# IvanPopov/video-flow-ml

Measured on AMD Instinct MI355X. Metric: flow-fields/sec @1080p seq5 MOF_sintel, higher is better.
Workload: dtype mixed (per-layer MFMA count, f32 accumulate): {"corr": 1, "update_block.encoder.convf1": 1, "update_block.encoder.convf2": 1, "update_block.gru.convq1.iter": "2a", "update_block.gru.convzr1.iter": 1, "update_block.gru.convzr2.iter": 1, "update_block.mask.0": 1, "update_block.mask.2": 1, "update_bloc

## Files before the change

include/vfml.h:

```cpp
#ifndef VFML_H
#define VFML_H
#include <stddef.h>
#include <stdint.h>

#ifdef __cplusplus
extern "C" {
#endif

#define VFML_ABI_VERSION 27

enum {
  VFML_EPI_NONE = 0,
  VFML_EPI_RELU = 1,
  VFML_EPI_TANH = 2,
  VFML_EPI_SIGMOID = 3,
  VFML_EPI_TANH_RELU = 4,
  VFML_EPI_GRU_ZR = 5,
  VFML_EPI_GRU_Q = 6,
  VFML_EPI_ADD_AUX = 7,
};

enum { VFML_FMT_F32 = 0, VFML_FMT_S16 = 1,
       VFML_FMT_F16 = 2 };

// ... 91 lines not shown
int vfml_avgpool2x2(const float* x, int n, int h, int w, int c, float* out, void* stream);

int vfml_corr_lookup(const float* const* pyr, const int32_t* hl, const int32_t* wl,
                     const int32_t* ld, int levels, int radius, int nmaps, int q_per_map,
                     const float* coords, int ld_coords, float* out, int ld_out, int out_fmt, int vol_fmt, int vol_tile,
                     void* stream);
#define VFML_VOL_F16_LEVELS(m) (0x100 | (m))

int vfml_corr_lookup_indirect(const float* const* table, const int32_t* hl, const int32_t* wl, const int32_t* ld,
                              int levels, int radius, int nmaps, int q_per_map, const float* coords, int ld_coords,
                              float* out, int ld_out, int out_fmt, int vol_fmt, int vol_tile, void* stream);
int vfml_corr_lookup_indirect_bidir(const float* const* table, const int32_t* hl, const int32_t* wl, const int32_t* ld,
                                    int levels, int radius, int nmaps, int q_per_map, const float* coords, int ld_coords,
                                    int dir_coords, float* out, int ld_out, int dir_out, int dir_tab, int out_fmt, int vol_fmt,
                                    int vol_tile, void* stream);
int vfml_ptr_table_set(void* table, const void* const* ptrs, int n, void* stream);

int vfml_corr_level0_ensure(const vfml_conv_desc* d, const void* w_hi, const void* w_lo, int kp, float w_scale, int in_fmt,
                            int out_fmt, int k_order, const void* const* cells, int centres, int dirs, int dir_cells,
                            const float* coords, int ld_coords, int dir_coords, int h, int w, int radius, int vol_tile,
                            uint32_t* counter, void* stream);

typedef struct vfml_corr_level_desc {
  const vfml_conv_desc* d;
  const void* w_hi;
  const void* w_lo;
  int32_t kp;
  float w_scale;
  int32_t out_fmt, level, h, w;
} vfml_corr_level_desc;
// ... 155 lines not shown
```

video-flow-ml_amd/vfml/csrc/flow_ops.hip:

```cpp
#include <stdlib.h>
#include "vfml_common.h"
#include "corr_window.h"

namespace {

constexpr int MAX_LEVELS = 6;
constexpr int MAX_MAPS = 8;
constexpr int MAX_RADIUS = 4;
constexpr int PATCH = 2 * MAX_RADIUS + 2;
#ifndef VFML_LOOKUP_WAVES
#define VFML_LOOKUP_WAVES 4
#endif
constexpr int LOOKUP_WAVES = VFML_LOOKUP_WAVES;
constexpr int FIXED_LEVELS = 4;
static_assert(FIXED_LEVELS == 4, "corr_lookup_fixed_kernel selects among four levels");

struct LookupArgs {
  const float* pyr[MAX_MAPS][MAX_LEVELS];
  const float* const* table;
  int hl[MAX_LEVELS], wl[MAX_LEVELS], ld[MAX_LEVELS];
  int levels, radius, nq, q_per_map;
  const float* coords; int ld_coords;
  float* out; int ld_out;
  int out16;
// ... 212 lines not shown
      for (int h = 0; h < 2; ++h) {
        const int c = lane * 8 + 4 * h;
        const f32x4 w = h ? v1 : v0;
        if (c + 3 < nout && (((uintptr_t)(o + 4 * h)) & 15u) == 0) {
          *reinterpret_cast<f32x4*>(o + 4 * h) = w;
        } else {
#pragma unroll
          for (int k = 0; k < 4; ++k)
            if (c + k < nout) o[4 * h + k] = w[k];
        }
      }
    }
  }
}

__global__ void coords_init_kernel(f32x4* __restrict__ coords, int h, int w, int64_t total) {
  for (int64_t p = (int64_t)blockIdx.x * blockDim.x + threadIdx.x; p < total; p += (int64_t)gridDim.x * blockDim.x) {
    const int x = (int)(p % w);
    const int y = (int)((p / w) % h);
    f32x4 v = {(float)x, (float)y, (float)x, (float)y};
    coords[p] = v;
  }
}

__global__ void flow_rows7_kernel(const f32x4* __restrict__ flow, int w, int64_t total, char* __restrict__ rows) {
  for (int64_t i = (int64_t)blockIdx.x * blockDim.x + threadIdx.x; i < total * 4; i += (int64_t)gridDim.x * blockDim.x) {
    const int64_t p = i >> 2;
    const int u = (int)(i & 3);
    const int x = (int)(p % w);
    f32x4 t0 = {0.f, 0.f, 0.f, 0.f}, t1 = {0.f, 0.f, 0.f, 0.f};
// ... 188 lines not shown
               "vfml_window_seed: rows >= 1, cols a multiple of 4, rows * cols / 4 <= 2^30");
  VFML_REQUIRE(ld_state % 4 == 0 && h_off >= 0 && mf_off >= 0 && h_off % 4 == 0 && mf_off % 4 == 0 && h_off + cols <= ld_state &&
               mf_off + cols <= ld_state && (h_off + cols <= mf_off || mf_off + cols <= h_off),
               "vfml_window_seed: the two column blocks lie apart inside a state row, at multiples of 4 floats");
  VFML_REQUIRE(ld_ctx >= cols && ld_ctx % 4 == 0, "vfml_window_seed: ld_ctx=%d (>= cols, a multiple of 4)", ld_ctx);
  const int quads = cols / 4;
  hipLaunchKernelGGL(window_seed_kernel, dim3(grid_for((int64_t)rows * quads, 256), ncentres), dim3(256), 0,
                     reinterpret_cast<hipStream_t>(stream), reinterpret_cast<const int64_t*>(cells), rows, quads, state,
                     ld_state, h_off, mf_off, ld_ctx);
  return vfml_check_launch("vfml_window_seed");
}

static int corr_lookup_impl(const float* const* pyr, const float* const* table, const int32_t* hl, const int32_t* wl,
                            const int32_t* ld, int levels, int radius, int nmaps, int q_per_map, const float* coords,
                            int ld_coords, float* out, int ld_out, int out_fmt, int vol_fmt, int vol_tile, void* stream,
                            int dir_maps = 0, int dir_coords = 0, int dir_out = 0, int dir_tab = 0);

extern "C" int vfml_corr_lookup(const float* const* pyr, const int32_t* hl, const int32_t* wl, const int32_t* ld,
                                int levels, int radius, int nmaps, int q_per_map, const float* coords, int ld_coords,
                                float* out, int ld_out, int out_fmt, int vol_fmt, int vol_tile, void* stream) {
  VFML_REQUIRE(pyr, "vfml_corr_lookup: null pointer");
  return corr_lookup_impl(pyr, nullptr, hl, wl, ld, levels, radius, nmaps, q_per_map, coords, ld_coords, out, ld_out, out_fmt,
                          vol_fmt, vol_tile, stream);
}

extern "C" int vfml_corr_lookup_indirect(const float* const* table, const int32_t* hl, const int32_t* wl, const int32_t* ld,
                                         int levels, int radius, int nmaps, int q_per_map, const float* coords,
                                         int ld_coords, float* out, int ld_out, int out_fmt, int vol_fmt, int vol_tile, void* stream) {
  VFML_REQUIRE(table && (reinterpret_cast<uintptr_t>(table) & 7u) == 0, "vfml_corr_lookup_indirect: null / misaligned table");
  return corr_lookup_impl(nullptr, table, hl, wl, ld, levels, radius, nmaps, q_per_map, coords, ld_coords, out, ld_out,
                          out_fmt, vol_fmt, vol_tile, stream);
// ... 1 lines not shown

extern "C" int vfml_corr_lookup_indirect_bidir(const float* const* table, const int32_t* hl, const int32_t* wl, const int32_t* ld,
                                               int levels, int radius, int nmaps, int q_per_map, const float* coords,
                                               int ld_coords, int dir_coords, float* out, int ld_out, int dir_out, int dir_tab,
                                               int out_fmt, int vol_fmt, int vol_tile, void* stream) {
  VFML_REQUIRE(table && (reinterpret_cast<uintptr_t>(table) & 7u) == 0, "vfml_corr_lookup_indirect_bidir: null / misaligned table");
  VFML_REQUIRE(nmaps >= 1 && 2 * nmaps <= MAX_MAPS, "vfml_corr_lookup_indirect_bidir: nmaps=%d out of [1,%d]", nmaps, MAX_MAPS / 2);
  VFML_REQUIRE(dir_coords >= 0 && dir_coords + 2 <= ld_coords && dir_out >= 0 && (out_fmt != VFML_FMT_S16 || dir_out % 8 == 0),
               "vfml_corr_lookup_indirect_bidir: dir_coords within a coords row, dir_out >= 0 (a multiple of 8 floats for split rows)");
  VFML_REQUIRE(dir_tab >= nmaps && (dir_tab + nmaps) * levels <= MAX_TABLE,
               "vfml_corr_lookup_indirect_bidir: dir_tab=%d (the second direction's first map in the table) out of range", dir_tab);
  return corr_lookup_impl(nullptr, table, hl, wl, ld, levels, radius, 2 * nmaps, q_per_map, coords, ld_coords, out, ld_out,
                          out_fmt, vol_fmt, vol_tile, stream, nmaps, dir_coords, dir_out, dir_tab);
}

static int corr_lookup_impl(const float* const* pyr, const float* const* table, const int32_t* hl, const int32_t* wl,
                            const int32_t* ld, int levels, int radius, int nmaps, int q_per_map, const float* coords,
                            int ld_coords, float* out, int ld_out, int out_fmt, int vol_fmt, int vol_tile, void* stream,
                            int dir_maps, int dir_coords, int dir_out, int dir_tab) {
  VFML_REQUIRE(nmaps >= 1 && nmaps <= MAX_MAPS && q_per_map > 0, "vfml_corr_lookup: nmaps=%d out of [1,%d] or empty maps", nmaps, MAX_MAPS);
  const int nq = nmaps * q_per_map;
  VFML_REQUIRE(out_fmt == VFML_FMT_F32 || out_fmt == VFML_FMT_S16, "vfml_corr_lookup: bad out_fmt");
  int v16mask = vol_fmt == VFML_FMT_F16 ? 15 : ((vol_fmt & ~15) == VFML_VOL_F16_LEVELS(0) ? (vol_fmt & 15) : (vol_fmt == VFML_FMT_F32 ? 0 : -1));
  if (v16mask > 0 && levels >= 1 && levels <= FIXED_LEVELS) {
    v16mask &= (1 << levels) - 1;
    if (v16mask) v16mask |= 15 & ~((1 << levels) - 1);
  }
  VFML_REQUIRE(v16mask == 0 || ((radius == 3 || radius == 4) && levels <= FIXED_LEVELS &&
                                (v16mask == 15 || v16mask == 14 || v16mask == 12 || v16mask == 8)),
               "vfml_corr_lookup: vol_fmt is VFML_FMT_F32, or (radius 3 / 4, at most %d levels) VFML_FMT_F16 or "
               "VFML_VOL_F16_LEVELS(m) with m = levels 1-3, 2-3 or 3", FIXED_LEVELS);
  VFML_REQUIRE(hl && wl && ld && coords && out, "vfml_corr_lookup: null pointer");
  VFML_REQUIRE(levels >= 1 && levels <= MAX_LEVELS, "vfml_corr_lookup: levels=%d out of [1,%d]", levels, MAX_LEVELS);
  VFML_REQUIRE(radius >= 1 && radius <= MAX_RADIUS, "vfml_corr_lookup: radius=%d out of [1,%d]", radius, MAX_RADIUS);
// ... 19 lines not shown
  }
  for (int l = levels; l < MAX_LEVELS; ++l) a.hl[l] = a.wl[l] = a.ld[l] = 0;
  a.tws = vol_tile & 15; a.ths = (vol_tile >> 4) & 15; a.qw = wl[0];
  VFML_REQUIRE(vol_tile >= 0 && vol_tile < 256 && a.tws <= 6 && a.ths <= 6, "vfml_corr_lookup: vol_tile = tws + 16 * ths with tws, ths <= 6");
  if (vol_tile) {
    VFML_REQUIRE(q_per_map == hl[0] * wl[0], "vfml_corr_lookup: a tiled volume orders its rows by the level-0 grid (q_per_map == hl[0] * wl[0])");
    for (int l = 0; l < levels; ++l)
      VFML_REQUIRE((int64_t)ld[l] >= (int64_t)(((hl[l] - 1) >> a.ths) + 1) * (((wl[l] - 1) >> a.tws) + 1) << (a.tws + a.ths),
                   "vfml_corr_lookup: ld[%d]=%d is less than the whole tiles of a %d x %d level", l, ld[l], wl[l], hl[l]);
  }
  a.levels = levels; a.radius = radius; a.nq = nq; a.q_per_map = q_per_map;
  a.coords = coords; a.ld_coords = ld_coords; a.out = out; a.ld_out = ld_out;
  a.dir_maps = dir_maps; a.dir_coords = dir_coords; a.dir_out = dir_out; a.dir_tab = dir_tab;
  const dim3 grid((nq + LOOKUP_WAVES - 1) / LOOKUP_WAVES), block(64 * LOOKUP_WAVES);
  hipStream_t st = reinterpret_cast<hipStream_t>(stream);
  if (a.vol16) {
    const int m = a.vol16;
#define VFML_LOOKUP16(RR, OO)                                                                                  \
  do {                                                                                                          \
    if (m == 15) hipLaunchKernelGGL((corr_lookup_fixed_kernel<RR, OO, 15>), grid, block, 0, st, a);             \
    else if (m == 14) hipLaunchKernelGGL((corr_lookup_fixed_kernel<RR, OO, 14>), grid, block, 0, st, a);        \
    else if (m == 12) hipLaunchKernelGGL((corr_lookup_fixed_kernel<RR, OO, 12>), grid, block, 0, st, a);        \
    else hipLaunchKernelGGL((corr_lookup_fixed_kernel<RR, OO, 8>), grid, block, 0, st, a);                      \
  } while (0)
    if (radius == 4) {
      if (a.out16) VFML_LOOKUP16(4, true);
      else VFML_LOOKUP16(4, false);
    } else {
      if (a.out16) VFML_LOOKUP16(3, true);
      else VFML_LOOKUP16(3, false);
// ... 169 lines not shown
```

video-flow-ml_amd/vfml/hip.py:

```python
import ctypes
import os
import subprocess
from ctypes import POINTER, c_char_p, c_double, c_float, c_int, c_int32, c_int64, c_void_p

import torch

_HERE = os.path.dirname(os.path.abspath(__file__))
LIB_PATH = os.environ.get("VFML_LIB") or os.path.join(_HERE, "libvfml_hip.so")
CSRC = os.path.join(_HERE, "csrc")
SOURCES = ["api.hip", "conv_gemm.hip", "conv_gemm_split.hip", "corr_ensure.hip", "conv_gemm_tapx.hip", "conv_split_plan.hip", "stem.hip", "flow_half.hip", "enc_conv.hip", "norm_pool.hip", "flow_ops.hip", "effects.hip", "correct.hip", "render.hip", "text.hip", "turbulence.hip", "resize.hip", "jpeg.hip", "jpeg_decode.hip", "jpeg_decode_sync.hip", "deflate.hip", "attention.hip", "dwconv.hip", "twins.hip", "warm_start.hip"]

STATS_ROWS_F32, STATS_ROWS_S16 = 128, 32
EPI_NONE, EPI_RELU, EPI_TANH, EPI_SIGMOID, EPI_TANH_RELU, EPI_GRU_ZR, EPI_GRU_Q, EPI_ADD_AUX = range(8)
FMT_F32, FMT_S16, FMT_F16 = 0, 1, 2


def vol_f16_levels(mask):
    return 0x100 | mask


def _vol_mask(vol_fmt, levels):
    return (15 if vol_fmt == FMT_F16 else (vol_fmt & 15 if vol_fmt & 0x100 else 0)) & ((1 << levels) - 1)

KORDER_TAP, KORDER_CBLOCK, KORDER_CBLOCK64 = 0, 1, 2
# ... 115 lines not shown
    L.vfml_instnorm_finalize.argtypes = [c_void_p, c_int, c_int, c_int, c_int, c_float, c_void_p, c_void_p, c_int64, c_void_p]
    L.vfml_instnorm_finalize_workspace_bytes.restype = c_int64
    L.vfml_instnorm_finalize_workspace_bytes.argtypes = [c_int, c_int]
    L.vfml_stem7x7s2_chunks.argtypes = [c_int, c_int]
    L.vfml_stem7x7s2.argtypes = [c_void_p, c_int, c_int, c_int, c_void_p, c_void_p, c_float, c_void_p, c_void_p, c_void_p, c_void_p]
    L.vfml_instnorm_apply.argtypes = [c_void_p, c_void_p, c_void_p, c_void_p, c_int, c_int, c_int, c_void_p, c_int, c_void_p]
    L.vfml_avgpool2x2.argtypes = [c_void_p, c_int, c_int, c_int, c_int, c_void_p, c_void_p]
    L.vfml_corr_lookup.argtypes = [POINTER(c_void_p), POINTER(c_int32), POINTER(c_int32), POINTER(c_int32),
                                   c_int, c_int, c_int, c_int, c_void_p, c_int, c_void_p, c_int, c_int, c_int, c_int, c_void_p]
    L.vfml_corr_lookup_indirect.argtypes = [c_void_p, POINTER(c_int32), POINTER(c_int32), POINTER(c_int32),
                                            c_int, c_int, c_int, c_int, c_void_p, c_int, c_void_p, c_int, c_int, c_int, c_int,
                                            c_void_p]
    L.vfml_corr_lookup_indirect_bidir.argtypes = [c_void_p, POINTER(c_int32), POINTER(c_int32), POINTER(c_int32),
                                                  c_int, c_int, c_int, c_int, c_void_p, c_int, c_int, c_void_p, c_int, c_int,
                                                  c_int, c_int, c_int, c_int, c_void_p]
    L.vfml_ptr_table_set.argtypes = [c_void_p, POINTER(c_void_p), c_int, c_void_p]
    L.vfml_corr_level0_ensure.argtypes = L.vfml_conv2d_split.argtypes[:5] + [c_int, c_int, c_int] + [
        c_void_p, c_int, c_int, c_int, c_void_p, c_int, c_int, c_int, c_int, c_int, c_int, c_void_p, c_void_p]
    L.vfml_corr_levels_ensure.argtypes = [POINTER(CorrLevelDesc), c_int, c_int, c_int, c_void_p, c_int, c_int, c_int, c_void_p,
                                          c_int, c_int, c_int, c_int, c_int, c_int, c_void_p, c_void_p]
    L.vfml_window_seed.argtypes = [c_void_p, c_int, c_int, c_int, c_void_p, c_int, c_int, c_int, c_int, c_void_p]
    L.vfml_tapsum3x3_update.argtypes = [c_void_p, c_int, c_void_p, c_int, c_int, c_int, c_int, ctypes.c_int64, c_void_p, c_void_p,
                                        c_int, c_void_p, c_int, c_int, c_void_p]
    L.vfml_conv3x3_c64.argtypes = [c_void_p, c_int, c_int, c_int, c_int, c_void_p, c_void_p, c_int, c_float, c_void_p, c_void_p,
                                   c_int, c_void_p, c_void_p]
    L.vfml_flow_half.argtypes = [c_void_p, c_int, c_int, c_int, c_void_p, c_int, c_float, c_void_p, c_void_p, c_int, c_float,
                                 c_void_p, c_void_p, c_int, c_void_p]
    L.vfml_coords_init.argtypes = [c_void_p, c_int, c_int, c_int, c_void_p]
    L.vfml_flow_rows7.argtypes = [c_void_p, c_int, c_int, c_int, c_void_p, c_void_p]
    L.vfml_tapsum3x3.argtypes = [c_void_p, c_int, c_void_p, c_int, c_int, c_int, c_void_p, c_int, ctypes.c_int64, c_void_p]
# ... 62 lines not shown
    L.vfml_inflate_chunks.argtypes = [c_void_p, c_int64, c_void_p, c_int, c_int, c_int64, ctypes.c_uint32, c_void_p, c_void_p,
                                      c_void_p, c_void_p, c_void_p]
    L.vfml_convex_upsample.argtypes = [c_void_p, c_int, c_void_p, c_int, c_int, c_int, c_void_p, c_void_p]
    for name in EXPORTS:
        getattr(L, name)
    if L.vfml_abi_version() != 27:
        raise RuntimeError("libvfml_hip.so ABI version mismatch")
    _lib = L
    return L


EXPORTS = [
    "vfml_conv2d", "vfml_conv2d_split", "vfml_conv2d_variant", "vfml_conv2d_split_variant", "vfml_conv2d_split_variant_at", "vfml_split_f16", "vfml_to_s16", "vfml_softmax_rows_s16", "vfml_softmax_rows_f16", "vfml_attention_plane_workspace_bytes", "vfml_attention_plane_f16", "vfml_attention_bank_planes_f16", "vfml_axpy_f32", "vfml_dwconv2d", "vfml_gelu_rows", "vfml_layernorm_rows", "vfml_window_attention", "vfml_attention_shared_keys", "vfml_transpose_to_s16", "vfml_add_to_s16",
    "vfml_transpose_split_f16", "vfml_frames_to_nhwc4", "vfml_instnorm_workspace_bytes", "vfml_instnorm_stats",
    "vfml_instnorm_apply", "vfml_instnorm_finalize", "vfml_instnorm_finalize_workspace_bytes", "vfml_avgpool2x2", "vfml_corr_lookup", "vfml_corr_lookup_indirect", "vfml_corr_lookup_indirect_bidir",
    "vfml_ptr_table_set", "vfml_corr_level0_ensure", "vfml_corr_levels_ensure", "vfml_window_seed", "vfml_coords_update", "vfml_coords_init", "vfml_tapsum3x3", "vfml_tapsum3x3_update", "vfml_flow_rows7", "vfml_flow_half", "vfml_conv3x3_c64",
    "vfml_flow_forward_interpolate_workspace_bytes", "vfml_flow_forward_interpolate",
    "vfml_convex_upsample", "vfml_stem7x7s2", "vfml_stem7x7s2_chunks", "vfml_flow_lod", "vfml_flow_encode", "vfml_taa_blend", "vfml_flow_quality_map", "vfml_flow_correct_workspace_bytes", "vfml_flow_correct",
    "vfml_flow_colorize", "vfml_compose_frame", "vfml_flow_decode", "vfml_flow_diff_overlay", "vfml_text_draw",
    "vfml_flow_turbulence_workspace_bytes", "vfml_flow_turbulence_map", "vfml_resize_u8",
    "vfml_jpeg_workspace_bytes", "vfml_jpeg_scan_capacity", "vfml_jpeg_encode_rgb",
    "vfml_jpeg_sampled_workspace_bytes", "vfml_jpeg_sampled_scan_capacity", "vfml_jpeg_encode_rgb_sampled",
    "vfml_jpeg_decode_workspace_bytes", "vfml_jpeg_decode_rgb",
    "vfml_jpeg_decode_sync_workspace_bytes", "vfml_jpeg_decode_rgb_sync",
    "vfml_jpeg_decode_sampled_workspace_bytes", "vfml_jpeg_decode_rgb_sampled",
    "vfml_jpeg_decode_sync_sampled_workspace_bytes", "vfml_jpeg_decode_rgb_sync_sampled",
    "vfml_deflate_capacity", "vfml_deflate_workspace_bytes", "vfml_deflate_huffman",
    "vfml_inflate_workspace_bytes", "vfml_inflate_chunks",
    "vfml_last_error", "vfml_abi_version",
]
# ... 415 lines not shown
        d.out, d.ldo = _ptr(_dev(volume)), ldo
        d.epilogue, d.split, d.out_scale = EPI_NONE, 0, out_scale
        d.flags = {3: 0, 2: CONV_MFMA2, 1: CONV_MFMA1}[mfma]
        lv = lvs[i]
        lv.d = ctypes.pointer(d)
        lv.w_hi, lv.w_lo, lv.kp, lv.w_scale = weight.hi.data_ptr(), weight.lo.data_ptr(), weight.kp, weight.scale
        lv.out_fmt, lv.level, lv.h, lv.w = FMT_F32, level, hl, wl
    order = levels[0][1].order
    _check(lib().vfml_corr_levels_ensure(lvs, len(levels), in_fmt, order, c_void_p(cells.data_ptr()), centres, ndirs, dir_cells,
                                         _ptr(_dev(coords), coords_off), ld_coords, dir_coords, h, w, radius, vol_tile,
                                         c_void_p(counters.data_ptr()) if counters is not None else None, _stream()),
           "vfml_corr_levels_ensure")


SEED_NONE, SEED_LOAD, SEED_STORE = 0, 1, 2


def window_seed(cells, ncentres, rows, cols, state, ld_state, h_off, mf_off, ld_ctx):
    if not (cells.is_cuda and cells.dtype == torch.int64 and cells.numel() >= 3 * ncentres):
        raise ValueError("window_seed: cells must be an int64 device tensor, three per centre frame")
    _check(lib().vfml_window_seed(c_void_p(cells.data_ptr()), ncentres, rows, cols, _ptr(_dev(state)), ld_state, h_off, mf_off,
                                  ld_ctx, _stream()), "vfml_window_seed")


def corr_lookup(pyrs, hl, wl, ld, radius, q_per_map, coords, coords_off, ld_coords, out, out_off, ld_out,
                out_fmt=FMT_F32, table=None, nmaps=None, vol_fmt=FMT_F32, vol_tile=0, bidir=None):
    L = len(hl)
    if bidir is not None:
        dir_coords, dir_out, dir_tab = bidir

        def launch():
            _check(lib().vfml_corr_lookup_indirect_bidir(c_void_p(table.data_ptr()), (c_int32 * L)(*hl), (c_int32 * L)(*wl),
                                                         (c_int32 * L)(*ld), L, radius, nmaps, q_per_map,
                                                         _ptr(_dev(coords), coords_off), ld_coords, dir_coords,
                                                         _ptr(_dev(out), out_off), ld_out, dir_out, dir_tab, out_fmt, vol_fmt,
                                                         vol_tile, _stream()), "vfml_corr_lookup_indirect_bidir")
    elif table is not None:
        def launch():
            _check(lib().vfml_corr_lookup_indirect(c_void_p(table.data_ptr()), (c_int32 * L)(*hl), (c_int32 * L)(*wl),
                                                   (c_int32 * L)(*ld), L, radius, nmaps, q_per_map,
                                                   _ptr(_dev(coords), coords_off), ld_coords, _ptr(_dev(out), out_off),
                                                   ld_out, out_fmt, vol_fmt, vol_tile, _stream()), "vfml_corr_lookup_indirect")
    else:
# ... 711 lines not shown
```

video-flow-ml_amd/vfml/network.py:

```python
import os
import types

import torch
import torch.nn as nn

from . import hip, update_block
from .weights import (BASE_CORR_LEVELS, BASE_CORR_RADIUS, GMA_NO_BIAS, TWINS_STAGES, TWINS_WS, conv_spec, corr_channel_subset,
                      is_depthwise, pack_conv_weight, pcblock_hidden, sk_blocks, twins_spec)

ATT_SCALE = 16384.0


def cor_pad(cor, split):
    return (cor + 15) // 16 * 16 if split else (cor + 3) // 4 * 4


def take_frames(src, idx):
    idx = list(idx)
    if all(b == a + 1 for a, b in zip(idx, idx[1:])):
        return src[idx[0]:idx[0] + len(idx)]
    return torch.stack([src[i] for i in idx])


class _Holder(nn.Module):
# ... 860 lines not shown
        v16 = [bool((mask >> l) & 1) for l in range(L)]
        VFl = [hip.FMT_F16 if v16[l] else hip.FMT_F32 for l in range(L)]
        VF = (hip.FMT_F32 if not mask else hip.FMT_F16 if mask == (1 << L) - 1 else hip.vol_f16_levels(mask))
        ldl = []
        for l in range(L):
            unit = 64 if v16[l] else 32
            n = (Nl[l] + unit - 1) // unit * unit
            ldl.append(n if (n // unit) % 2 else n + unit)
        psz = [(Pv * ldl[l] + 1) // 2 if v16[l] else Pv * ldl[l] for l in range(L)]
        return types.SimpleNamespace(L=L, AF=AF, hl=hl, wl=wl, Sl=Sl, VT=VT, Nl=Nl, Pv=Pv, TILE=TILE, vol16=mask, VF=VF,
                                     VFl=VFl, ldl=ldl, psz=psz)

    corr_on_demand = True
    corr_on_demand_levels = (1,)

    def _corr_scale(self, AF):
        scale = 1.0 / float(self.cfg.feat_dim) ** 0.5
        if AF == hip.FMT_S16:
            scale /= self.FMAP_ROW_SCALE
        return scale

    def _level0_on_demand(self, keys, N, geo, dense_corr=False):
        return (self.corr_on_demand and not dense_corr and keys is not None and self._split() and not self.tri_frame
                and not self.gma and not self.sk and geo.AF == hip.FMT_S16 and geo.Pv % 4 == 0 and geo.Nl[0] >= 1024
                and geo.VT is not None and geo.Pv == geo.Nl[0] and geo.VFl[0] == hip.FMT_F32 and self._nm("corr") == 1
                and self.cfg.feat_dim <= 256 and 2 * (N - 2) <= 8 and (geo.Nl[0] + 63) // 64 <= 2048)

    def _on_demand_levels(self, on_demand, geo):
        if not on_demand:
            return ()
# ... 263 lines not shown

    def _iteration(self, s, win, it, ng, nm, branch):
        ub = update_block
        ne, r0 = (1, (win.M - 1) * s.Pn) if win.warm and it == 0 else (nm, 0)
        join = None
        if branch is not None:
            fork = torch.cuda.Event()
            fork.record()
            with torch.cuda.stream(branch):
                branch.wait_event(fork)
                ub.flow_half(s, ne, r0)
                join = torch.cuda.Event()
                join.record()
        if win.ensure is not None:
            ub.ensure_level0(s, ne, r0, win.ensure)
        ub.lookup(s, ne, r0, win.tables, win.bidir)
        ub.convc1(s, ne, r0)
        ub.convc2(s, ne, r0)
        if join is None:
            ub.flow_half(s, ne, r0)
        else:
            torch.cuda.current_stream(win.dev).wait_event(join)
        ub.encoder_conv(s, ne, r0)
        if it == 0:
            hip.window_seed(win.seed_cells, win.M, s.Pn, 128, s.G, s.GLD, s.HH, s.MF, 256)
        if self.gma:
            self._gma_readout(s, win, ng)
        update_block.temporal_fusion(s, win.M if self.tri_frame else nm, stack=not self.tri_frame)
        ub.sep_conv_gru(s, ng, *win.gates)
        ub.flow_head(s, ng)

# ... 54 lines not shown
            pyrs = self._window_pyramids(feats, keys, N, geo, dev, od_levels)
            s = self._window_state(P, dev, M, h, w, geo, R, AF, cor_p)
            ctx = self._frame_context(src, list(range(1, N - 1)), keys, H, W, P, dev, Pn, M)
            win = types.SimpleNamespace(M=M, dev=dev, att_slots=(), readout=None)
            if self.gma:
                att = self._att_store
                win.att_slots = tuple(ctx[c][4] for c in range(1, N - 1))
                att["live"] = set(win.att_slots)
                win.readout = update_block.readout_scratch(self._buf, dev, MP, Pn, self.ATT_DIM, att["ldA"], att["plain"],
                                                           att["vt"])
            it0, win.warm, it0_new, win.seed_cells = self._seed_plan(s, ctx, keys, dev, M, R, pick_only)
            win.gates = self._gate_addends(ctx, dev, Pn, M)
            win.sk_ws = self._sk_workspace(MP, dev) if self.sk else None
            win.tables, win.bidir = self._pyramid_tables(pyrs, dev, M, L, cor_p)
            win.ensure = self._ensure_plan(pyrs, feats, N, geo, dev, od_levels) if on_demand else None
            no, nflows = (1, 1) if short else (M, 2 * M)
            up_fixed = self._buf("up_out", nflows * H * W * 2, dev)
            mask = self._buf("mask", MP * 1152, dev)

            def body():
                update_block.init_coords(s, M)
                branch = None
                if os.environ.get("VFML_FLOW_BRANCH", "0") == "1" and self._split():
                    branch = self._side2.get(dev)
                    if branch is None:
                        branch = self._side2[dev] = torch.cuda.Stream(device=dev)
                if self.sk:
                    hip.window_seed(win.seed_cells, M, Pn, 256, s.G, s.GLD, s.HH, s.MF, 256)
                for it in range(cfg.decoder_depth):
                    left = cfg.decoder_depth - 1 - it
                    ng = min(M, left + 1) if short else M
                    nm = min(M, left + 2) if short else M
                    if self.sk:
                        self._sk_iteration(s, win, ng, nm)
                    else:
                        self._iteration(s, win, it, ng, nm, branch)
                if cfg.decoder_depth == 0 and not self.sk:
                    hip.window_seed(win.seed_cells, M, Pn, 128, s.G, s.GLD, s.HH, s.MF, 256)
                update_block.mask_head(s, no, mask, 1152)
                if short:
                    hip.convex_upsample(s.coords1, 0, 2, mask, 576, 1152, h, w, up_fixed)
                else:
                    for d in range(2):
                        for c in range(M):
                            hip.convex_upsample(s.coords1, c * Pn * 4, 2 * d, mask, c * Pn * 1152 + d * 576, 1152, h, w,
                                                up_fixed, out_off=(d * M + c) * H * W * 2)

            gkey = (H, W, N, M, bool(tri_batch), bool(pick_only), cfg.decoder_depth, L, R, self._plan_key(), geo.vol16, od_levels,
                    self._packed_serial, str(dev), os.environ.get("VFML_FLOW_BRANCH", "0"), win.warm, win.att_slots, on_demand)
            if self.sk:
                gkey += ("sk",)
            self._pre_body = torch.cuda.Event()
            self._pre_body.record(torch.cuda.current_stream(dev))
            try:
                self._run_body(body, gkey, dev)
            except BaseException:
                if it0_new:
                    it0["ring"].forget(it0_new)
                raise
            up = up_fixed.clone().view(nflows, H, W, 2)
            flow = up.permute(0, 3, 1, 2).unsqueeze(0)
            if short:
                return flow, None
            low = s.flow4.view(M, h, w, 4)[..., :].clone() if return_lowres else None
# ... 6 lines not shown
```

video-flow-ml_amd/vfml/update_block.py:

```python
import types

from . import hip

UB = "update_block"


def window_state(P, nm, AF, h, w, geo, R, G, GLD, cols, ld_corr, cor_p, rows7, tapsum, **maps):
    return types.SimpleNamespace(P=P, nm=nm, AF=AF, h=h, w=w, Pn=h * w, geo=geo, R=R, G=G, GLD=GLD, ld_corr=ld_corr, cor_p=cor_p,
                                 rows7=rows7, tapsum=tapsum,
                                 fuse=AF == hip.FMT_S16,
                                 **cols, **maps)


def _put_flow(s):
    return dict(flow_a=s.flow4, ld_a=4, flow_b=s.G, ld_b=s.GLD, flow_b_off=s.MF + 124, fmt_b=s.AF)


def init_coords(s, n, flow_init=None):
    hip.coords_init(s.coords1, n, s.h, s.w)
    hip.coords_update(s.coords1, flow_init, n, s.h, s.w, **_put_flow(s))


def lookup(s, n, r0, tables=(), bidir=None, pyrs=None):
    g = s.geo
    if pyrs is not None:
        hip.corr_lookup(pyrs, g.hl, g.wl, g.ldl, s.R, s.Pn, s.coords1, r0 * 4, 4, s.corr, r0 * s.ld_corr, s.ld_corr,
                        out_fmt=s.AF, vol_fmt=g.VF, vol_tile=g.TILE)
        return
    t0 = r0 // s.Pn * g.L
    for d, tab in enumerate(tables):
        hip.corr_lookup(None, g.hl, g.wl, g.ldl, s.R, s.Pn, s.coords1, r0 * 4 + 2 * d, 4, s.corr, r0 * s.ld_corr + d * s.cor_p,
                        s.ld_corr, out_fmt=s.AF, table=tab[t0:], nmaps=n, vol_fmt=g.VF, vol_tile=g.TILE, bidir=bidir)


def ensure_level0(s, n, r0, en):
    g = s.geo
    c0 = r0 // s.Pn
    hip.corr_levels_ensure(en.rows, en.D, g.Pv, en.levels, en.scale, en.cells[en.per * c0:], n, 2, en.M, s.coords1, r0 * 4, 4, 2,
                           g.hl[0], g.wl[0], s.R, g.TILE, counters=en.counter, in_fmt=s.AF)


def convc1(s, n, r0):
    wgt, b = s.P[f"{UB}.encoder.convc1"]
    hip.conv2d(s.corr, s.ld_corr, s.ld_corr, n, s.h, s.w, wgt, b, 256, 1, 1, s.c1, 256, epilogue=hip.EPI_RELU,
               in0_off=r0 * s.ld_corr, out_off=r0 * 256, in_fmt=s.AF, out_fmt=s.AF, mfma=s.nm(f"{UB}.encoder.convc1"))


# ... 127 lines not shown
```

Before: 49.26.

## Cache correlation lookup patches across GRU iterations keyed by window origins

Result: faster. 50.35 (median of 6 runs) (+2.2%).

```diff
diff --git a/include/vfml.h b/include/vfml.h
--- a/include/vfml.h
+++ b/include/vfml.h
@@ -129,6 +129,11 @@
                                     int levels, int radius, int nmaps, int q_per_map, const float* coords, int ld_coords,
                                     int dir_coords, float* out, int ld_out, int dir_out, int dir_tab, int out_fmt, int vol_fmt,
                                     int vol_tile, void* stream);
+int vfml_corr_lookup_indirect_bidir_cached(const float* const* table, const int32_t* hl, const int32_t* wl, const int32_t* ld,
+                                           int levels, int radius, int nmaps, int q_per_map, const float* coords,
+                                           int ld_coords, int dir_coords, float* out, int ld_out, int dir_out, int dir_tab,
+                                           int out_fmt, int vol_fmt, int vol_tile, float* cache, int32_t* key, int cache_rows,
+                                           int row0, int store, uint32_t* counter, void* stream);
 int vfml_ptr_table_set(void* table, const void* const* ptrs, int n, void* stream);
 
 int vfml_corr_level0_ensure(const vfml_conv_desc* d, const void* w_hi, const void* w_lo, int kp, float w_scale, int in_fmt,
diff --git a/video-flow-ml_amd/vfml/csrc/flow_ops.hip b/video-flow-ml_amd/vfml/csrc/flow_ops.hip
--- a/video-flow-ml_amd/vfml/csrc/flow_ops.hip
+++ b/video-flow-ml_amd/vfml/csrc/flow_ops.hip
@@ -250,6 +250,167 @@
   }
 }
 
+struct LookupCache {
+  float* patch;
+  int* key;
+  int rows, row0;
+  int store;
+  unsigned* counter;
+};
+
+template <int R, bool OUT16, int V16 = 0>
+__global__ __launch_bounds__(64 * LOOKUP_WAVES) void corr_lookup_fixed_cached_kernel(const LookupArgs a, const LookupCache c) {
+  constexpr int SIDE = 2 * R + 2, PSZ = SIDE * SIDE, WIN = 2 * R + 1, WW = WIN * WIN;
+  constexpr int NOUTPAD = (FIXED_LEVELS * WW + 7) & ~7;
+  static_assert(PSZ <= 128 && FIXED_LEVELS * WIN <= 64 && NOUTPAD / 8 <= 64, "one wave: at most two gather passes per level");
+  static_assert(PSZ % 4 == 0 && FIXED_LEVELS * PSZ <= 4 * 128, "a patch moves as at most two 16-byte quads per lane");
+  __shared__ __attribute__((aligned(16))) float patch[LOOKUP_WAVES][FIXED_LEVELS][PSZ];
+  __shared__ __attribute__((aligned(16))) float outs[LOOKUP_WAVES][NOUTPAD];
+  const int lane = threadIdx.x & 63;
+  const int wv = __builtin_amdgcn_readfirstlane(threadIdx.x >> 6);
+  const int q = blockIdx.x * LOOKUP_WAVES + wv;
+  if (q >= a.nq) return;
+  int map = __builtin_amdgcn_readfirstlane(q / a.q_per_map);
+  const int qq = q - map * a.q_per_map;
+  const int qrow = __builtin_amdgcn_readfirstlane((a.tws | a.ths) ? tiled_at(qq / a.qw, qq % a.qw, a.qw, a.tws, a.ths) : qq);
+  int64_t crow, orow;
+  const int qdir = a.dir_maps && map >= a.dir_maps;
+  const int64_t krow = (int64_t)qdir * c.rows + c.row0 + (q - (qdir ? a.dir_maps * a.q_per_map : 0));
+  lookup_rows(a, q, map, crow, orow);
+  const float cx = a.coords[crow + 0];
+  const float cy = a.coords[crow + 1];
+  int ox[FIXED_LEVELS], oy[FIXED_LEVELS];
+#pragma unroll
+  for (int l = 0; l < FIXED_LEVELS; ++l) {
+    ox[l] = window_origin(level_coord(cx, l), R);
+    oy[l] = window_origin(level_coord(cy, l), R);
+  }
+  const int4* kp = reinterpret_cast<const int4*>(c.key + krow * (2 * FIXED_LEVELS));
+  const int4 k0 = kp[0], k1 = kp[1];
+  const bool same = k0.x == ox[0] && k0.y == oy[0] && k0.z == ox[1] && k0.w == oy[1] &&
+                    k1.x == ox[2] && k1.y == oy[2] && k1.z == ox[3] && k1.w == oy[3];
+  const bool hit = __builtin_amdgcn_readfirstlane(same ? 1 : 0) != 0;
+  if (hit) {
+    const f32x4* src = reinterpret_cast<const f32x4*>(c.patch + krow * (FIXED_LEVELS * PSZ));
+    f32x4* dst = reinterpret_cast<f32x4*>(&patch[wv][0][0]);
+    if (4 * lane < a.levels * PSZ) dst[lane] = src[lane];
+    if (4 * (lane + 64) < a.levels * PSZ) dst[lane + 64] = src[lane + 64];
+  } else {
+    const int pyA = lane / SIDE, pxA = lane - pyA * SIDE;
+    const int pyB = (lane + 64) / SIDE, pxB = (lane + 64) - pyB * SIDE;
+    const bool inB = lane + 64 < PSZ;
+    const float* pl[FIXED_LEVELS];
+    if (a.table) {
+#pragma unroll
+      for (int l = 0; l < FIXED_LEVELS; ++l) pl[l] = a.table[map * a.levels + (l < a.levels ? l : 0)];
+    } else {
+#pragma unroll
+      for (int l = 0; l < FIXED_LEVELS; ++l) pl[l] = a.pyr[map][l < a.levels ? l : 0];
+    }
+    float va[FIXED_LEVELS], vb[FIXED_LEVELS];
+    bool oka[FIXED_LEVELS], okb[FIXED_LEVELS];
+#pragma unroll
+    for (int l = 0; l < FIXED_LEVELS; ++l) {
+      const bool have = l < a.levels;
+      const int ll = have ? l : 0;
+      const bool v16 = (V16 >> l) & 1;
+      const int ES = v16 ? 2 : 4;
+      const char* base = reinterpret_cast<const char*>(pl[l]) + (int64_t)qrow * a.ld[ll] * ES;
+      const int wl = a.wl[ll], hl = a.hl[ll];
+      const float x = level_coord(cx, l), y = level_coord(cy, l);
+      const int x0 = window_origin(x, R);
+      const int y0 = window_origin(y, R);
+      auto texel = [&](int px, int py, bool in, float& out, bool& ok) {
+        const int xx = x0 + px, yy = y0 + py;
+        ok = have && in && xx >= 0 && xx < wl && yy >= 0 && yy < hl;
+        const int at = tiled_at(min(max(yy, 0), hl - 1), min(max(xx, 0), wl - 1), wl, a.tws, a.ths);
+        if (v16) out = (float)((const __attribute__((address_space(1))) _Float16*)base)[at];
+        else out = ((const __attribute__((address_space(1))) float*)base)[at];
+      };
+      texel(pxA, pyA, true, va[l], oka[l]);
+      if constexpr (PSZ > 64) texel(pxB, pyB, inB, vb[l], okb[l]);
+      else { vb[l] = 0.f; okb[l] = false; }
+    }
+#pragma unroll
+    for (int l = 0; l < FIXED_LEVELS; ++l) {
+      va[l] = oka[l] ? va[l] : 0.f;
+      vb[l] = okb[l] ? vb[l] : 0.f;
+    }
+#pragma unroll
+    for (int l = 0; l < FIXED_LEVELS; ++l) {
+      if (l < a.levels) {
+        if (PSZ > 64 || lane < PSZ) patch[wv][l][lane] = va[l];
+        if constexpr (PSZ > 64) if (inB) patch[wv][l][lane + 64] = vb[l];
+      }
+    }
+  }
+  const int nout = a.levels * WW;
+  const int nunits = (nout + 7) >> 3;
+  if (lane >= 56 && nout + (lane - 56) < nunits * 8) outs[wv][nout + (lane - 56)] = 0.f;
+  wave_lds_sync();
+  if (!hit && c.store) {
+    f32x4* dst = reinterpret_cast<f32x4*>(c.patch + krow * (FIXED_LEVELS * PSZ));
+    const f32x4* src = reinterpret_cast<const f32x4*>(&patch[wv][0][0]);
+    if (4 * lane < a.levels * PSZ) dst[lane] = src[lane];
+    if (4 * (lane + 64) < a.levels * PSZ) dst[lane + 64] = src[lane + 64];
+    if (lane == 0) {
+      int4* kq = reinterpret_cast<int4*>(c.key + krow * (2 * FIXED_LEVELS));
+      kq[0] = make_int4(ox[0], oy[0], ox[1], oy[1]);
+      kq[1] = make_int4(ox[2], oy[2], ox[3], oy[3]);
+    }
+  }
+  if (c.counter && lane == 0) atomicAdd(c.counter + (hit ? 0 : 1), 1u);
+  if (lane < a.levels * WIN) {
+    const int l = lane / WIN, i = lane - l * WIN;
+    const float x = level_coord(cx, l), y = level_coord(cy, l);
+    const float fx = x - floorf(x), fy = y - floorf(y);
+    const float wx0 = 1.f - fx, wy0 = 1.f - fy;
+    const float w00 = wx0 * wy0, w10 = fx * wy0, w01 = wx0 * fy, w11 = fx * fy;
+    const float* p = &patch[wv][l][i];
+    float* o = &outs[wv][l * WW + i * WIN];
+    float nw = p[0], ne = p[1];
+#pragma unroll
+    for (int j = 0; j < WIN; ++j) {
+      const float sw = p[(j + 1) * SIDE], se = p[(j + 1) * SIDE + 1];
+      o[j] = bilinear4w(nw, ne, sw, se, w00, w10, w01, w11);
+      nw = sw; ne = se;
+    }
+  }
+  wave_lds_sync();
+  if (lane < nunits) {
+    float* o = a.out + orow + lane * 8;
+    const f32x4 v0 = *reinterpret_cast<const f32x4*>(&outs[wv][lane * 8]);
+    const f32x4 v1 = *reinterpret_cast<const f32x4*>(&outs[wv][lane * 8 + 4]);
+    if (OUT16) {
+      vfml_h16x2 h0, h1, h2, h3, l0, l1, l2, l3;
+      vfml_split2(v0[0], v0[1], h0, l0);
+      vfml_split2(v0[2], v0[3], h1, l1);
+      vfml_split2(v1[0], v1[1], h2, l2);
+      vfml_split2(v1[2], v1[3], h3, l3);
+      uint4 hv, lv;
+      hv.x = __builtin_bit_cast(unsigned, h0); hv.y = __builtin_bit_cast(unsigned, h1);
+      hv.z = __builtin_bit_cast(unsigned, h2); hv.w = __builtin_bit_cast(unsigned, h3);
+      lv.x = __builtin_bit_cast(unsigned, l0); lv.y = __builtin_bit_cast(unsigned, l1);
+      lv.z = __builtin_bit_cast(unsigned, l2); lv.w = __builtin_bit_cast(unsigned, l3);
+      *reinterpret_cast<uint4*>(o) = hv;
+      *reinterpret_cast<uint4*>(o + 4) = lv;
+    } else {
+#pragma unroll
+      for (int h = 0; h < 2; ++h) {
+        const int c = lane * 8 + 4 * h;
+        const f32x4 w = h ? v1 : v0;
+        if (c + 3 < nout && (((uintptr_t)(o + 4 * h)) & 15u) == 0) {
+          *reinterpret_cast<f32x4*>(o + 4 * h) = w;
+        } else {
+#pragma unroll
+          for (int k = 0; k < 4; ++k)
+            if (c + k < nout) o[4 * h + k] = w[k];
+        }
+      }
+    }
+  }
+}
+
 __global__ void coords_init_kernel(f32x4* __restrict__ coords, int h, int w, int64_t total) {
   for (int64_t p = (int64_t)blockIdx.x * blockDim.x + threadIdx.x; p < total; p += (int64_t)gridDim.x * blockDim.x) {
     const int x = (int)(p % w);
@@ -468,7 +629,8 @@
 static int corr_lookup_impl(const float* const* pyr, const float* const* table, const int32_t* hl, const int32_t* wl,
                             const int32_t* ld, int levels, int radius, int nmaps, int q_per_map, const float* coords,
                             int ld_coords, float* out, int ld_out, int out_fmt, int vol_fmt, int vol_tile, void* stream,
-                            int dir_maps = 0, int dir_coords = 0, int dir_out = 0, int dir_tab = 0);
+                            int dir_maps = 0, int dir_coords = 0, int dir_out = 0, int dir_tab = 0,
+                            const LookupCache* cache = nullptr);
 
 extern "C" int vfml_corr_lookup(const float* const* pyr, const int32_t* hl, const int32_t* wl, const int32_t* ld,
                                 int levels, int radius, int nmaps, int q_per_map, const float* coords, int ld_coords,
@@ -500,10 +662,37 @@
                           out_fmt, vol_fmt, vol_tile, stream, nmaps, dir_coords, dir_out, dir_tab);
 }
 
+extern "C" int vfml_corr_lookup_indirect_bidir_cached(const float* const* table, const int32_t* hl, const int32_t* wl,
+                                                      const int32_t* ld, int levels, int radius, int nmaps, int q_per_map,
+                                                      const float* coords, int ld_coords, int dir_coords, float* out, int ld_out,
+                                                      int dir_out, int dir_tab, int out_fmt, int vol_fmt, int vol_tile,
+                                                      float* cache, int32_t* key, int cache_rows, int row0, int store,
+                                                      uint32_t* counter, void* stream) {
+  const char* me = "vfml_corr_lookup_indirect_bidir_cached";
+  VFML_REQUIRE(table && (reinterpret_cast<uintptr_t>(table) & 7u) == 0, "%s: null / misaligned table", me);
+  VFML_REQUIRE(nmaps >= 1 && 2 * nmaps <= MAX_MAPS, "%s: nmaps=%d out of [1,%d]", me, nmaps, MAX_MAPS / 2);
+  VFML_REQUIRE(dir_coords >= 0 && dir_coords + 2 <= ld_coords && dir_out >= 0 && (out_fmt != VFML_FMT_S16 || dir_out % 8 == 0),
+               "%s: dir_coords within a coords row, dir_out >= 0 (a multiple of 8 floats for split rows)", me);
+  VFML_REQUIRE(dir_tab >= nmaps && levels >= 1 && (dir_tab + nmaps) * levels <= MAX_TABLE,
+               "%s: dir_tab=%d (the second direction's first map in the table) out of range", me, dir_tab);
+  VFML_REQUIRE((radius == 3 || radius == 4) && levels <= FIXED_LEVELS,
+               "%s: radius=%d, levels=%d - the patch cache belongs to the fixed-radius kernels (radius 3 or 4, at most %d levels)",
+               me, radius, levels, FIXED_LEVELS);
+  VFML_REQUIRE(cache && key, "%s: null cache / key", me);
+  VFML_REQUIRE(vfml_aligned16(cache) && vfml_aligned16(key), "%s: cache and key rows must be 16-byte aligned", me);
+  VFML_REQUIRE(q_per_map > 0 && row0 >= 0 && cache_rows >= 1 && (int64_t)row0 + (int64_t)nmaps * q_per_map <= cache_rows,
+               "%s: rows %d .. +%d x %d outside the cache's %d rows per direction", me, row0, nmaps, q_per_map, cache_rows);
+  VFML_REQUIRE(counter == nullptr || (reinterpret_cast<uintptr_t>(counter) & 3u) == 0, "%s: misaligned counter", me);
+  LookupCache c;
+  c.patch = cache; c.key = key; c.rows = cache_rows; c.row0 = row0; c.store = store != 0; c.counter = counter;
+  return corr_lookup_impl(nullptr, table, hl, wl, ld, levels, radius, 2 * nmaps, q_per_map, coords, ld_coords, out, ld_out,
+                          out_fmt, vol_fmt, vol_tile, stream, nmaps, dir_coords, dir_out, dir_tab, &c);
+}
+
 static int corr_lookup_impl(const float* const* pyr, const float* const* table, const int32_t* hl, const int32_t* wl,
                             const int32_t* ld, int levels, int radius, int nmaps, int q_per_map, const float* coords,
                             int ld_coords, float* out, int ld_out, int out_fmt, int vol_fmt, int vol_tile, void* stream,
-                            int dir_maps, int dir_coords, int dir_out, int dir_tab) {
+                            int dir_maps, int dir_coords, int dir_out, int dir_tab, const LookupCache* cache) {
   VFML_REQUIRE(nmaps >= 1 && nmaps <= MAX_MAPS && q_per_map > 0, "vfml_corr_lookup: nmaps=%d out of [1,%d] or empty maps", nmaps, MAX_MAPS);
   const int nq = nmaps * q_per_map;
   VFML_REQUIRE(out_fmt == VFML_FMT_F32 || out_fmt == VFML_FMT_S16, "vfml_corr_lookup: bad out_fmt");
@@ -553,6 +742,27 @@
   a.dir_maps = dir_maps; a.dir_coords = dir_coords; a.dir_out = dir_out; a.dir_tab = dir_tab;
   const dim3 grid((nq + LOOKUP_WAVES - 1) / LOOKUP_WAVES), block(64 * LOOKUP_WAVES);
   hipStream_t st = reinterpret_cast<hipStream_t>(stream);
+  if (cache) {
+    const LookupCache c = *cache;
+    const int m = a.vol16;
+#define VFML_LOOKUP_CACHED(RR, OO)                                                                                  \
+  do {                                                                                                               \
+    if (m == 15) hipLaunchKernelGGL((corr_lookup_fixed_cached_kernel<RR, OO, 15>), grid, block, 0, st, a, c);        \
+    else if (m == 14) hipLaunchKernelGGL((corr_lookup_fixed_cached_kernel<RR, OO, 14>), grid, block, 0, st, a, c);   \
+    else if (m == 12) hipLaunchKernelGGL((corr_lookup_fixed_cached_kernel<RR, OO, 12>), grid, block, 0, st, a, c);   \
+    else if (m == 8) hipLaunchKernelGGL((corr_lookup_fixed_cached_kernel<RR, OO, 8>), grid, block, 0, st, a, c);     \
+    else hipLaunchKernelGGL((corr_lookup_fixed_cached_kernel<RR, OO, 0>), grid, block, 0, st, a, c);                 \
+  } while (0)
+    if (radius == 4) {
+      if (a.out16) VFML_LOOKUP_CACHED(4, true);
+      else VFML_LOOKUP_CACHED(4, false);
+    } else {
+      if (a.out16) VFML_LOOKUP_CACHED(3, true);
+      else VFML_LOOKUP_CACHED(3, false);
+    }
+#undef VFML_LOOKUP_CACHED
+    return vfml_check_launch("vfml_corr_lookup_indirect_bidir_cached");
+  }
   if (a.vol16) {
     const int m = a.vol16;
 #define VFML_LOOKUP16(RR, OO)                                                                                  \
diff --git a/video-flow-ml_amd/vfml/hip.py b/video-flow-ml_amd/vfml/hip.py
--- a/video-flow-ml_amd/vfml/hip.py
+++ b/video-flow-ml_amd/vfml/hip.py
@@ -153,6 +153,8 @@
     L.vfml_corr_lookup_indirect_bidir.argtypes = [c_void_p, POINTER(c_int32), POINTER(c_int32), POINTER(c_int32),
                                                   c_int, c_int, c_int, c_int, c_void_p, c_int, c_int, c_void_p, c_int, c_int,
                                                   c_int, c_int, c_int, c_int, c_void_p]
+    L.vfml_corr_lookup_indirect_bidir_cached.argtypes = L.vfml_corr_lookup_indirect_bidir.argtypes[:-1] + [
+        c_void_p, c_void_p, c_int, c_int, c_int, c_void_p, c_void_p]
     L.vfml_ptr_table_set.argtypes = [c_void_p, POINTER(c_void_p), c_int, c_void_p]
     L.vfml_corr_level0_ensure.argtypes = L.vfml_conv2d_split.argtypes[:5] + [c_int, c_int, c_int] + [
         c_void_p, c_int, c_int, c_int, c_void_p, c_int, c_int, c_int, c_int, c_int, c_int, c_void_p, c_void_p]
@@ -245,6 +247,7 @@
     "vfml_conv2d", "vfml_conv2d_split", "vfml_conv2d_variant", "vfml_conv2d_split_variant", "vfml_conv2d_split_variant_at", "vfml_split_f16", "vfml_to_s16", "vfml_softmax_rows_s16", "vfml_softmax_rows_f16", "vfml_attention_plane_workspace_bytes", "vfml_attention_plane_f16", "vfml_attention_bank_planes_f16", "vfml_axpy_f32", "vfml_dwconv2d", "vfml_gelu_rows", "vfml_layernorm_rows", "vfml_window_attention", "vfml_attention_shared_keys", "vfml_transpose_to_s16", "vfml_add_to_s16",
     "vfml_transpose_split_f16", "vfml_frames_to_nhwc4", "vfml_instnorm_workspace_bytes", "vfml_instnorm_stats",
     "vfml_instnorm_apply", "vfml_instnorm_finalize", "vfml_instnorm_finalize_workspace_bytes", "vfml_avgpool2x2", "vfml_corr_lookup", "vfml_corr_lookup_indirect", "vfml_corr_lookup_indirect_bidir",
+    "vfml_corr_lookup_indirect_bidir_cached",
     "vfml_ptr_table_set", "vfml_corr_level0_ensure", "vfml_corr_levels_ensure", "vfml_window_seed", "vfml_coords_update", "vfml_coords_init", "vfml_tapsum3x3", "vfml_tapsum3x3_update", "vfml_flow_rows7", "vfml_flow_half", "vfml_conv3x3_c64",
     "vfml_flow_forward_interpolate_workspace_bytes", "vfml_flow_forward_interpolate",
     "vfml_convex_upsample", "vfml_stem7x7s2", "vfml_stem7x7s2_chunks", "vfml_flow_lod", "vfml_flow_encode", "vfml_taa_blend", "vfml_flow_quality_map", "vfml_flow_correct_workspace_bytes", "vfml_flow_correct",
@@ -690,6 +693,7 @@
 
 
 SEED_NONE, SEED_LOAD, SEED_STORE = 0, 1, 2
+LOOKUP_KEY_NONE = -2 ** 31
 
 
 def window_seed(cells, ncentres, rows, cols, state, ld_state, h_off, mf_off, ld_ctx):
@@ -700,9 +704,27 @@
 
 
 def corr_lookup(pyrs, hl, wl, ld, radius, q_per_map, coords, coords_off, ld_coords, out, out_off, ld_out,
-                out_fmt=FMT_F32, table=None, nmaps=None, vol_fmt=FMT_F32, vol_tile=0, bidir=None):
+                out_fmt=FMT_F32, table=None, nmaps=None, vol_fmt=FMT_F32, vol_tile=0, bidir=None, cache=None):
     L = len(hl)
-    if bidir is not None:
+    if cache is not None:
+        if bidir is None or table is None:
+            raise ValueError("corr_lookup: the patch cache goes with the bidirectional table lookup")
+        dir_coords, dir_out, dir_tab = bidir
+        patches, keys, rows, row0, store, counter = cache
+        if keys.dtype != torch.int32 or (counter is not None and counter.dtype != torch.int32):
+            raise ValueError("corr_lookup: cache keys and counter are int32 device tensors")
+        side = 2 * radius + 2
+        if patches.numel() < 2 * rows * 4 * side * side or keys.numel() < 2 * rows * 8:
+            raise ValueError(f"corr_lookup: cache of {patches.numel()} floats / {keys.numel()} keys is too small for 2 x {rows} rows")
+
+        def launch():
+            _check(lib().vfml_corr_lookup_indirect_bidir_cached(
+                c_void_p(table.data_ptr()), (c_int32 * L)(*hl), (c_int32 * L)(*wl), (c_int32 * L)(*ld), L, radius, nmaps,
+                q_per_map, _ptr(_dev(coords), coords_off), ld_coords, dir_coords, _ptr(_dev(out), out_off), ld_out, dir_out,
+                dir_tab, out_fmt, vol_fmt, vol_tile, _ptr(_dev(patches)), c_void_p(_dev(keys, torch.int32).data_ptr()), rows,
+                row0, int(bool(store)), c_void_p(counter.data_ptr()) if counter is not None else None, _stream()),
+                "vfml_corr_lookup_indirect_bidir_cached")
+    elif bidir is not None:
         dir_coords, dir_out, dir_tab = bidir
 
         def launch():
diff --git a/video-flow-ml_amd/vfml/network.py b/video-flow-ml_amd/vfml/network.py
--- a/video-flow-ml_amd/vfml/network.py
+++ b/video-flow-ml_amd/vfml/network.py
@@ -898,6 +898,29 @@
     corr_on_demand = True
     corr_on_demand_levels = (1,)
 
+    lookup_cache = True
+    lookup_cache_count = False
+
+    def _lookup_cache_plan(self, win, s, M, L, R, dev):
+        if not (self.lookup_cache and win.bidir is not None and self._split() and not self.sk and not self.tri_frame
+                and R in (3, 4) and L == 4):
+            return None
+        rows = M * s.Pn
+        counts = None
+        if self.lookup_cache_count:
+            counts = self._buf("lookup_count", 2 * max(1, self.cfg.decoder_depth), dev, torch.int32, zero=True)
+        return (self._buf("lookup_patches", 2 * rows * 4 * (2 * R + 2) ** 2, dev),
+                self._buf("lookup_keys", 2 * rows * 8, dev, torch.int32), rows, counts)
+
+    def lookup_cache_counts(self, reset=True):
+        count = self._ws.get("lookup_count")
+        if count is None:
+            return []
+        n = [int(v) for v in count.tolist()]
+        if reset:
+            count.zero_()
+        return list(zip(n[0::2], n[1::2]))
+
     def _corr_scale(self, AF):
         scale = 1.0 / float(self.cfg.feat_dim) ** 0.5
         if AF == hip.FMT_S16:
@@ -1191,7 +1214,11 @@
                 join.record()
         if win.ensure is not None:
             ub.ensure_level0(s, ne, r0, win.ensure)
-        ub.lookup(s, ne, r0, win.tables, win.bidir)
+        cache = None
+        if win.cache is not None:
+            patches, keys, rows, counts = win.cache
+            cache = (patches, keys, rows, it + 1 < self.cfg.decoder_depth, counts[2 * it:] if counts is not None else None)
+        ub.lookup(s, ne, r0, win.tables, win.bidir, cache=cache)
         ub.convc1(s, ne, r0)
         ub.convc2(s, ne, r0)
         if join is None:
@@ -1276,12 +1303,15 @@
             win.sk_ws = self._sk_workspace(MP, dev) if self.sk else None
             win.tables, win.bidir = self._pyramid_tables(pyrs, dev, M, L, cor_p)
             win.ensure = self._ensure_plan(pyrs, feats, N, geo, dev, od_levels) if on_demand else None
+            win.cache = self._lookup_cache_plan(win, s, M, L, R, dev)
             no, nflows = (1, 1) if short else (M, 2 * M)
             up_fixed = self._buf("up_out", nflows * H * W * 2, dev)
             mask = self._buf("mask", MP * 1152, dev)
 
             def body():
                 update_block.init_coords(s, M)
+                if win.cache is not None:
+                    win.cache[1].fill_(hip.LOOKUP_KEY_NONE)
                 branch = None
                 if os.environ.get("VFML_FLOW_BRANCH", "0") == "1" and self._split():
                     branch = self._side2.get(dev)
@@ -1309,7 +1339,9 @@
                                                 up_fixed, out_off=(d * M + c) * H * W * 2)
 
             gkey = (H, W, N, M, bool(tri_batch), bool(pick_only), cfg.decoder_depth, L, R, self._plan_key(), geo.vol16, od_levels,
-                    self._packed_serial, str(dev), os.environ.get("VFML_FLOW_BRANCH", "0"), win.warm, win.att_slots, on_demand)
+                    self._packed_serial, str(dev), os.environ.get("VFML_FLOW_BRANCH", "0"),
+                    win.cache is not None, win.cache is not None and win.cache[3] is not None,
+                    win.warm, win.att_slots, on_demand)
             if self.sk:
                 gkey += ("sk",)
             self._pre_body = torch.cuda.Event()
diff --git a/video-flow-ml_amd/vfml/update_block.py b/video-flow-ml_amd/vfml/update_block.py
--- a/video-flow-ml_amd/vfml/update_block.py
+++ b/video-flow-ml_amd/vfml/update_block.py
@@ -21,7 +21,7 @@
     hip.coords_update(s.coords1, flow_init, n, s.h, s.w, **_put_flow(s))
 
 
-def lookup(s, n, r0, tables=(), bidir=None, pyrs=None):
+def lookup(s, n, r0, tables=(), bidir=None, pyrs=None, cache=None):
     g = s.geo
     if pyrs is not None:
         hip.corr_lookup(pyrs, g.hl, g.wl, g.ldl, s.R, s.Pn, s.coords1, r0 * 4, 4, s.corr, r0 * s.ld_corr, s.ld_corr,
@@ -30,7 +30,8 @@
     t0 = r0 // s.Pn * g.L
     for d, tab in enumerate(tables):
         hip.corr_lookup(None, g.hl, g.wl, g.ldl, s.R, s.Pn, s.coords1, r0 * 4 + 2 * d, 4, s.corr, r0 * s.ld_corr + d * s.cor_p,
-                        s.ld_corr, out_fmt=s.AF, table=tab[t0:], nmaps=n, vol_fmt=g.VF, vol_tile=g.TILE, bidir=bidir)
+                        s.ld_corr, out_fmt=s.AF, table=tab[t0:], nmaps=n, vol_fmt=g.VF, vol_tile=g.TILE, bidir=bidir,
+                        cache=cache[:3] + (r0,) + cache[3:] if cache is not None else None)
 
 
 def ensure_level0(s, n, r0, en):
```
